# LY-zhang-yi-hao/ORB-SLAM3_byZyh

Hardware: AMD Instinct MI355X
Metric: ORB features/ms (640x480, 8-level) + LocalBA iter ms @1/2/4/8 GPU (higher is better)
Workload: dtype u8; 1 GPU; C2: batch of 64 synthetic 640x480 frames per GPU, nFeatures=1000, 8 levels, extraction+description (ORBextractor::operator()); frames_per_gpu=64, width=640, height=480, nfeatures=1000, nlevels=8, batches_in_flight=4, parallelism=frame-sharded x1

## Files before the change

### orb-slam3_byzyh_amd/csrc/orb_extract.hip

```cpp
#include <hip/hip_ext.h>
#include <hip/hip_runtime.h>

#include <algorithm>
#include <cstdio>
#include <cstdlib>
#include <cstring>
#include <mutex>
#include <string>
#include <type_traits>
#include <vector>

#include "orb_extract_geom.h"
#include "orb_hd.h"
#include "orb_sincos.h"
#include "orbgpu.h"
#include "orbgpu_internal.h"

using namespace orbgpu;

namespace {

constexpr int kPatternSrc[1024] = {
#include "orb_pattern31.inc"
};
// ... 1327 lines not shown

template <bool kKeysInLds>
__device__ void qt2_run(QT2& T, uint32_t* keys, uint16_t* node, int K, int N, int nroots, float root_w, int span_y,
                        const uint32_t* __restrict__ cand_level, const CellDesc* __restrict__ cells, int cell_begin,
                        int cell_count, const int32_t* __restrict__ ccount, int n_first, int slot_first,
                        uint32_t* __restrict__ sel_out, int sel_cap, int* n_sel, int* status, int debug_flags,
                        unsigned long long* stamps, const QPlace& place) {
    QTree& t = T.t;
    const int tid = threadIdx.x, lane = tid & 63, wave = tid >> 6, lcap = t.lcap;
    int* ctrl = T.ctrl;
    unsigned long long* tm = ((debug_flags & 4) && stamps && tid == 0) ? stamps : nullptr;
    if (tm)
        for (int i = 0; i < kQtStamps; ++i) tm[i] = 0;
    unsigned long long t_last = tm ? __builtin_amdgcn_s_memtime() : 0;
    auto stamp = [&](int i) {
        if (tm) { const unsigned long long now = __builtin_amdgcn_s_memtime(); tm[i] += now - t_last; t_last = now; }
    };
    int rcount[kMaxRoots];
#pragma unroll
    for (int r = 0; r < kMaxRoots; ++r) rcount[r] = 0;
    {
        constexpr int kGB = 8;
        int carry = 0;
        for (int cb = 0; cb < cell_count; cb += kQtThreads) {
            const int c = cb + tid;
            int n = 0, slot = 0;
            if (cb == 0) { n = n_first; slot = slot_first; }
            else if (c < cell_count) { n = ccount[c]; slot = cells[cell_begin + c].slot; }
            const int incl = wave_incl_scan(n, lane);
            const int start = incl - n;
            const int Tw = uniform(__builtin_amdgcn_readlane(incl, 63));
            if (lane == 0) ctrl[24 + wave] = Tw;
            __syncthreads();
            int base = carry, tot = 0;
#pragma unroll
            for (int w = 0; w < kQtWaves; ++w) {
                const int v = ctrl[24 + w];
                base += w < wave ? v : 0;
                tot += v;
            }
            __syncthreads();
            for (int j0 = 0; j0 < Tw; j0 += 64 * kGB) {
                uint32_t kk[kGB];
#pragma unroll
                for (int gi = 0; gi < kGB; ++gi) {
                    const int i = j0 + 64 * gi + lane;
                    int cl = 0;
#pragma unroll
                    for (int s = 32; s > 0; s >>= 1)
                        if (__shfl(start, cl + s, 64) <= i) cl += s;
                    const int sl = __shfl(slot, cl, 64), s0 = __shfl(start, cl, 64);
                    kk[gi] = i < Tw ? cand_level[sl + (i - s0)] : 0u;
                }
#pragma unroll
                for (int gi = 0; gi < kGB; ++gi) {
                    const int i = j0 + 64 * gi + lane;
                    if (i < Tw) {
                        int root = 0;
                        if (nroots > 1) {
                            root = (int)((float)key_x(kk[gi]) / root_w);
#pragma unroll
                            for (int r = 0; r < kMaxRoots; ++r) rcount[r] += root == r;
                        }
                        keys[base + i] = kk[gi];
                        node[base + i] = (uint16_t)root;
                    }
                }
            }
            carry += tot;
        }
    }
    if (tid < kMaxRoots) ctrl[16 + tid] = 0;
    __syncthreads();
    if (nroots > 1) {
#pragma unroll
        for (int r = 0; r < kMaxRoots; ++r) {
            if (r >= nroots) break;
            const int s = wave_sum(rcount[r]);
            if (lane == 0 && s) atomicAdd(&ctrl[16 + r], s);
        }
    } else if (tid == 0) {
        ctrl[16] = K;
    }
    __syncthreads();
    stamp(0);
    QGen A = t.g0, B = t.g1;
    int32_t* cA = T.cnt[0];
    int32_t* cB = T.cnt[1];
    uint32_t* sA = T.sxy[0];
    uint32_t* sB = T.sxy[1];
    int nlist = 0;
    if (tid == 0) {
        for (int r = 0; r < nroots; ++r) {
            const int n = ctrl[16 + r];
            if (n > 0) {
                const int x0 = (int)(root_w * (float)r), x1 = (int)(root_w * (float)(r + 1));
                A.x0[nlist] = (int16_t)x0; A.x1[nlist] = (int16_t)x1;
                A.y0[nlist] = 0; A.y1[nlist] = (int16_t)span_y;
                A.kn[nlist] = n; A.leaf[nlist] = n == 1;
                sA[nlist] = n > 1 ? qt2_split_word(x0, 0, x1, span_y) : ~0u;
#pragma unroll
                for (int q = 0; q < 4; ++q) cA[q * lcap + nlist] = 0;
                ctrl[8 + r] = nlist;
                nlist++;
            }
        }
        ctrl[2] = nlist;
    }
    __syncthreads();
    nlist = ctrl[2];
    for (int kb = wave * 64; kb < K; kb += kQtThreads) {
        const int k = kb + lane;
        int p = 0, q = 0;
        bool counted = false;
        if (k < K) {
            if (nroots > 1) {
                p = ctrl[8 + node[k]];
                node[k] = (uint16_t)p;
            }
            const uint32_t s = sA[p];
            counted = s != ~0u;
            q = qt2_quadrant(keys[k], s);
        }
        if (counted) atomicAdd(&cA[q * lcap + p], 1);
    }
    __syncthreads();
    stamp(1);
    bool careful = false, fin = false, ovf = false;
    int nsplit = 0;
    while (true) {
        if (wave == 0) {
            int new_size = 0;
            if (!careful) {
                qt2_regular(T, A, B, cA, cB, sB, nlist, N, lane, new_size, nsplit, fin, ovf);
                if (!fin && !ovf && new_size + nsplit * 3 > N) careful = true;
                stamp(2);
                if (tm) tm[9]++;
            } else {
                if (tm) tm[8] += (unsigned long long)nsplit << (16 * min((int)tm[10], 3));
                qt2_careful(T, A, B, cA, cB, sB, nlist, nsplit, N, lane, debug_flags, K < (1 << 20), new_size, nsplit, fin, ovf, tm,
                            t_last);
                stamp(5);
                if (tm) tm[10]++;
            }
            nlist = new_size;
            if (lane == 0) { ctrl[0] = fin; ctrl[1] = ovf; }
        }
        __syncthreads();
        fin = ctrl[0] != 0;
        ovf = ctrl[1] != 0;
        if (ovf) break;
        for (int kb = wave * 128; kb < K; kb += 2 * kQtThreads) {
            const int k0 = kb + lane, k1 = kb + 64 + lane;
            const bool v0 = k0 < K, v1 = k1 < K;
            const int p0 = v0 ? node[k0] : 0, p1 = v1 ? node[k1] : 0;
            const uint32_t key0 = v0 ? keys[k0] : 0u, key1 = v1 ? keys[k1] : 0u;
            const uint32_t s0 = sA[p0], s1 = sA[p1];
            const unsigned long long m0 = T.cmap[p0], m1 = T.cmap[p1];
            const int n0 = (int)((m0 >> (16 * qt2_quadrant(key0, s0))) & 0xffff);
            const int n1 = (int)((m1 >> (16 * qt2_quadrant(key1, s1))) & 0xffff);
            if (v0) node[k0] = (uint16_t)n0;
            if (v1) node[k1] = (uint16_t)n1;
            if (fin) {
                if (v0) atomicMax(&T.best[n0], ((uint32_t)key_score(key0) << 24) | (0xffffffu - (uint32_t)k0));
                if (v1) atomicMax(&T.best[n1], ((uint32_t)key_score(key1) << 24) | (0xffffffu - (uint32_t)k1));
            } else {
                const uint32_t t0 = v0 ? sB[n0] : ~0u, t1 = v1 ? sB[n1] : ~0u;
                if (t0 != ~0u) atomicAdd(&cB[qt2_quadrant(key0, t0) * lcap + n0], 1);
                if (t1 != ~0u) atomicAdd(&cB[qt2_quadrant(key1, t1) * lcap + n1], 1);
            }
        }
        __syncthreads();
        stamp(careful && !fin ? 6 : 3);
        { const QGen g = A; A = B; B = g; }
        { int32_t* c = cA; cA = cB; cB = c; }
        { uint32_t* s = sA; sA = sB; sB = s; }
        if (fin) break;
    }
    if (wave != 0) return;
    if (ovf || nlist > sel_cap) {
        if (lane == 0) { *n_sel = 0; atomicMax(status, 1); }
        return;
    }
    int carry_lap = 0, carry_mono = 0;
    for (int b = 0; b < nlist; b += 64) {
        const int i = b + lane;
        bool lap = false;
        if (i < nlist) {
            const uint32_t bw = T.best[i];
            const uint32_t best = keys[0xffffffu - (bw & 0xffffffu)];
            sel_out[i] = best;
            float x = (float)(key_x(best) + place.minB);
            if (place.level != 0) x = x * place.scale;
            lap = x >= (float)place.lap0 && x <= (float)place.lap1;
        }
        const unsigned long long ml = ballot(i < nlist && lap), mm = ballot(i < nlist && !lap);
        if (i < nlist) place.rank_out[i] = lap ? -(1 + carry_lap + rank_in(ml)) : carry_mono + rank_in(mm);
        carry_lap += __popcll(ml);
        carry_mono += __popcll(mm);
    }
    if (lane == 0) { *n_sel = nlist; *place.n_lap = carry_lap; }
    stamp(7);
    if (tm) tm[11] = (unsigned long long)K;
}

__global__ __launch_bounds__(kQtThreads) void k_quadtree_kp(
    const KernelGeom* __restrict__ gp, const CellDesc* __restrict__ cells, const uint32_t* __restrict__ cand,
    const int32_t* __restrict__ cell_count, uint32_t* __restrict__ key_scratch, uint32_t* __restrict__ sel,
    int32_t* __restrict__ sel_count, int lds_bytes, int* __restrict__ status, unsigned long long* __restrict__ stamps,
    int lap0, int lap1, int32_t* __restrict__ rank_out, int32_t* __restrict__ lap_count, int level0) {
    const KernelGeom& g = *gp;
    extern __shared__ __attribute__((aligned(16))) uint8_t smem[];
    const int level = level0 + blockIdx.x, f = blockIdx.y, tid = threadIdx.x, lane = tid & 63, wave = tid >> 6;
    const LevelGeom& L = g.lv[level];
    const int32_t* cc = cell_count + (size_t)f * g.ncells + L.cell_begin;
    int32_t* n_sel = sel_count + (size_t)f * g.nlevels + level;
    const int lcap = L.sel_cap + 64;
    const size_t meta = (qt2_meta_bytes(lcap) + 15) & ~(size_t)15;
    if (meta > (size_t)lds_bytes) {
        if (tid == 0) { *n_sel = 0; atomicMax(status, 2); }
        return;
    }
    QT2 T;
    qt2_carve(T, smem, lcap);
    int n_first = 0, slot_first = 0, Kp = 0;
    for (int c = tid; c < L.cell_count; c += kQtThreads) {
        const int v = cc[c];
        if (c == tid) { n_first = v; slot_first = cells[L.cell_begin + c].slot; }
        Kp += v;
    }
    Kp = wave_sum(Kp);
    if (lane == 0) T.ctrl[24 + kQtWaves + wave] = Kp;
    __syncthreads();
    int K = 0;
#pragma unroll
    for (int w = 0; w < kQtWaves; ++w) K += T.ctrl[24 + kQtWaves + w];
    uint32_t* sel_out = sel + (size_t)f * g.sel_frame_cap + L.sel_off;
    const uint32_t* cand_level = cand + (size_t)f * g.cand_frame_cap + L.cand_off;
    QPlace place{level, L.minB, lap0, lap1, L.scale, rank_out + (size_t)f * g.sel_frame_cap + L.sel_off,
                 lap_count + (size_t)f * g.nlevels + level};
    unsigned long long* st = stamps ? stamps + ((size_t)f * g.nlevels + level) * kQtStamps : nullptr;
    if (!(g.debug_flags & 8) && meta + (size_t)K * 6 <= (size_t)lds_bytes) {
        uint32_t* keys = (uint32_t*)(smem + meta);
        uint16_t* node = (uint16_t*)(keys + K);
        qt2_run<true>(T, keys, node, K, L.nfeat, L.n_roots, L.root_w, L.maxBY - L.minB, cand_level, cells,
                      L.cell_begin, L.cell_count, cc, n_first, slot_first, sel_out, L.sel_cap, n_sel, status,
                      g.debug_flags, st, place);
    } else {
        uint32_t* keys = key_scratch + ((size_t)f * g.cand_frame_cap + L.cand_off) * 2;
        uint16_t* node = (uint16_t*)(keys + L.cand_cap);
        qt2_run<false>(T, keys, node, K, L.nfeat, L.n_roots, L.root_w, L.maxBY - L.minB, cand_level, cells,
                       L.cell_begin, L.cell_count, cc, n_first, slot_first, sel_out, L.sel_cap, n_sel, status,
                       g.debug_flags, st, place);
    }
}

__global__ __launch_bounds__(64) void k_debug_node_sort(const int* __restrict__ counts, const int* __restrict__ ulx,
                                                        int n, int mode, int* __restrict__ order, int* __restrict__ used_reg) {
    extern __shared__ __attribute__((aligned(16))) uint8_t smem[];
    QT2 T;
    qt2_carve(T, smem, n + 64);
    QTree& t = T.t;
    QGen& A = t.g0;
    const int lane = threadIdx.x;
    for (int i = lane; i < n; i += 64) { A.kn[i] = counts[i]; A.x0[i] = (int16_t)ulx[i]; t.prev[i] = (uint16_t)i; }
    wave_sync();
    const bool reg = mode == 0 && n <= 64 && qt_sort_reg(t, A, n, lane);
    if (!reg) qt_sort(t, A, n, lane);
    for (int i = lane; i < n; i += 64) order[i] = t.prev[i];
    if (lane == 0) *used_reg = reg;
}

constexpr int kExcPerLane = (kNumSincosExc + 31) / 32;
template <bool kLds = false>
__device__ __forceinline__ void steer_sincos(float ang, const uint32_t (&exc)[kExcPerLane], int half, int hl,
                                             float* s, float* c, const uint2* lds_cs = nullptr) {
    orb_det_sincosf(ang, s, c);
    const uint32_t bits = __float_as_uint(ang);
    int idx = -1;
#pragma unroll
    for (int e = 0; e < kExcPerLane; ++e)
        if (32 * e + hl < kNumSincosExc && exc[e] == bits) idx = 32 * e + hl;
    const uint32_t hm = (uint32_t)(ballot(idx >= 0) >> (32 * (half & 1)));
    if (hm) {
        const int hit = __shfl(idx, 32 * (half & 1) + __builtin_ctz(hm), 64);
        if constexpr (kLds) {
            *c = __uint_as_float(lds_cs[hit].x);
            *s = __uint_as_float(lds_cs[hit].y);
        } else {
            *c = __uint_as_float(c_sincos_exc[hit][1]);
            *s = __uint_as_float(c_sincos_exc[hit][2]);
        }
    }
}

constexpr int kDescKpPerBlock = 8;
constexpr int kPR = 43, kPRW = 12;
constexpr int kHP = 22, kHPW = 40;
constexpr int kDescWords = kHP * kHPW;
static_assert(kDescWords >= (kPR + 1) * kPRW + 1, "patch + the last pair's odd row and over-read word fit the region");

typedef float f32x2 __attribute__((ext_vector_type(2)));
constexpr f32x2 kRound2 = {12582912.0f, 12582912.0f};
constexpr int kRoundBits = 0x4B400000;

__device__ __forceinline__ int blur_sample(const uint32_t* __restrict__ H, int r, int c) {
    const unsigned i = (unsigned)(r + 18) & 63u, cc = (unsigned)(c + 18) & 63u;
    const uint32_t* p = H + __umul24(i >> 1, (unsigned)kHPW) + cc;
    const bool odd = (i & 1) != 0;
    uint32_t acc = 1u << 15;
    acc = __builtin_amdgcn_udot2(as_u16x2(p[0]), odd ? w16(0, 18) : w16(18, 34), acc, false);
    acc = __builtin_amdgcn_udot2(as_u16x2(p[kHPW]), odd ? w16(34, 48) : w16(48, 56), acc, false);
    acc = __builtin_amdgcn_udot2(as_u16x2(p[2 * kHPW]), odd ? w16(56, 48) : w16(48, 34), acc, false);
    acc = __builtin_amdgcn_udot2(as_u16x2(p[3 * kHPW]), odd ? w16(34, 18) : w16(18, 0), acc, false);
    return (int)(acc >> 16);
}

__global__ __launch_bounds__(256) void k_describe(const KernelGeom* __restrict__ gp, const uint8_t* __restrict__ pyr,
                                                  const uint32_t* __restrict__ sel,
                                                  const int32_t* __restrict__ sel_count,
                                                  const int32_t* __restrict__ rank_in_class, const int32_t* __restrict__ lap_count,
                                                  int cap, orb_keypoint_t* __restrict__ kps, uint8_t* __restrict__ desc,
                                                  int32_t* __restrict__ counts, int chunks, int nblocks, int share,
                                                  int stage_levels, int stage_mode, orb_keypoint_t* __restrict__ st_kp,
                                                  uint8_t* __restrict__ st_desc) {
    const KernelGeom& g = *gp;
    __shared__ __attribute__((aligned(16))) uint32_t patch[kDescKpPerBlock][kDescWords];
    const int half = threadIdx.x >> 5, hl = threadIdx.x & 31;
    const int tb = xcd_tile(blockIdx.x, share);
    if (tb >= nblocks) return;
    const int f = tb / chunks, chunk0 = tb - f * chunks;
    int level = 0, chunk = chunk0;
#pragma unroll
    for (int l = 0; l + 1 < kMaxLevels; ++l) {
        const int c = (g.lv[l].sel_cap + kDescKpPerBlock - 1) / kDescKpPerBlock;
        if (l + 1 < g.nlevels && level == l && chunk >= c) { chunk -= c; level = l + 1; }
    }
    const int slot = chunk * kDescKpPerBlock + half;
    const LevelGeom& L = g.lv[level];
    const size_t sbase = (size_t)f * g.sel_frame_cap + L.sel_off + (slot < L.sel_cap ? slot : L.sel_cap - 1);
    const uint32_t key_spec = L.sel_cap > 0 ? sel[sbase] : 0u;
    const int rk_spec = L.sel_cap > 0 ? rank_in_class[sbase] : 0;
    const int li = hl & 15;
    const int cnt_l = li < g.nlevels ? sel_count[(size_t)f * g.nlevels + li] : 0;
    const int lap_l = li < g.nlevels ? lap_count[(size_t)f * g.nlevels + li] : 0;
    uint32_t pat[8], exc[kExcPerLane], disc[16];
#pragma unroll
    for (int m = 0; m < 8; ++m) pat[m] = c_pattern_packed.w[32 * m + hl];
#pragma unroll
    for (int m = 0; m < 16; ++m) disc[m] = c_disc.w[hl][m];
#pragma unroll
    for (int e = 0; e < kExcPerLane; ++e) exc[e] = 32 * e + hl < kNumSincosExc ? c_sincos_exc[32 * e + hl][0] : 0u;
    int total = cnt_l, lap_before = li < level ? lap_l : 0, mono_before = li < level ? cnt_l - lap_l : 0;
    total = row16_isum(total);
    lap_before = row16_isum(lap_before);
    mono_before = row16_isum(mono_before);
    const int n = __shfl(cnt_l, (threadIdx.x & ~15) + level, 64);
    const size_t st_idx = sbase;
    if (stage_mode != 1 && chunk0 == 0 && threadIdx.x == 0) {
        int mono = 0;
        for (int l = 0; l < g.nlevels; ++l)
            mono += sel_count[(size_t)f * g.nlevels + l] - lap_count[(size_t)f * g.nlevels + l];
        counts[2 * f] = total;
        counts[2 * f + 1] = total > cap ? ORB_ERR_CAPACITY : mono;
    }
    if (chunk * kDescKpPerBlock >= n) return;
    const bool active = slot < n && (stage_mode == 1 || total <= cap);
    if (stage_mode == 2 && level < stage_levels) {
        if (!active) return;
        const int rk = rk_spec;
        const int dst = rk < 0 ? total - 1 - (lap_before + (-rk - 1)) : mono_before + rk;
        if (hl < 8)
            reinterpret_cast<uint32_t*>(desc + ((size_t)f * cap + dst) * 32)[hl] =
                reinterpret_cast<const uint32_t*>(st_desc + st_idx * 32)[hl];
        else if (hl == 8)
            kps[(size_t)f * cap + dst] = st_kp[st_idx];
        return;
    }
    const uint32_t key = active ? key_spec : 0;
    const int x = key_x(key) + L.minB, y = key_y(key) + L.minB;
    constexpr int kGroups = (kPR + 9) / 10;
    const int pr = hl / 3, pq = hl - 3 * pr;
    const uint8_t* up = pyr + (size_t)f * g.pyr_frame_bytes + L.plane_off;
    const int po = (y + kEdge - 21) * L.pitch + (x + kEdge - 21);
    const int sh = po & 3;
    const uint32_t vo = (uint32_t)(po - sh + pr * L.pitch + 16 * pq);
    const __amdgpu_buffer_rsrc_t ru = __builtin_amdgcn_make_buffer_rsrc(const_cast<uint8_t*>(up), (short)0, 0x7fffffff, kBufDword3);
    uint32_t* P = patch[half];
    if (active && hl < 30) {
        v4u32 v[kGroups];
#pragma unroll
        for (int k = 0; k < kGroups; ++k) v[k] = __builtin_amdgcn_raw_buffer_load_b128(ru, vo, 10 * k * L.pitch, 0);
#pragma unroll
        for (int k = 0; k < kGroups; ++k)
            if (10 * k + pr < kPR) *reinterpret_cast<v4u32*>(P + (10 * k + pr) * kPRW + 4 * pq) = v[k];
    }
    wave_sync();
    int m10 = 0, m01 = 0;
    {
        const int rb = sh + (hl + 6) * (kPRW * 4) + 6;
        const uint32_t* rw = P + (rb >> 2);
        const int ra = rb & 3;
        uint32_t d[9];
#pragma unroll
        for (int k = 0; k < 9; ++k) d[k] = rw[k];
        uint32_t S = 0, W = 0;
#pragma unroll
        for (int k = 0; k < 8; ++k) {
            const uint32_t x = __builtin_amdgcn_alignbyte(d[k + 1], d[k], ra);
            S = __builtin_amdgcn_udot4(x, disc[k], S, false);
            W = __builtin_amdgcn_udot4(x, disc[8 + k], W, false);
        }
        if (active && hl < 31) {
            m01 = (hl - 15) * (int)S;
            m10 = (int)W - 16 * (int)S;
        }
    }
    m10 = half_wave_sum(m10);
    m01 = half_wave_sum(m01);
    const float angle = orb_fast_atan2((float)m01, (float)m10);
    constexpr int kItems = kHP * 10, kIt = (kItems + 31) / 32;
#pragma unroll
    for (int it = kIt - 1; it >= 0; --it) {
        const int i = hl + 32 * it, ic = min(i, kItems - 1), j = ic / 10, qq = ic - 10 * j;
        uint32_t o[2][4];
#pragma unroll
        for (int rr = 0; rr < 2; ++rr) {
            const uint32_t* w = P + (2 * j + rr) * kPRW + qq;
            const uint32_t w0 = w[0], w1 = w[1], w2 = w[2], w3 = w[3];
            const uint32_t a0 = __builtin_amdgcn_alignbyte(w1, w0, sh);
            const uint32_t a1 = __builtin_amdgcn_alignbyte(w2, w1, sh);
            const uint32_t a2 = __builtin_amdgcn_alignbyte(w3, w2, sh);
            o[rr][0] = __builtin_amdgcn_udot4(a1, kBlurK1, __builtin_amdgcn_udot4(a0, kBlurK0, 0u, false), false);
            o[rr][1] = __builtin_amdgcn_udot4(a1, kBlurS1[1], __builtin_amdgcn_udot4(a0, kBlurS0[1], 0u, false), false);
            o[rr][2] = __builtin_amdgcn_udot4(a2, kBlurS2[2], __builtin_amdgcn_udot4(a1, kBlurS1[2],
                                              __builtin_amdgcn_udot4(a0, kBlurS0[2], 0u, false), false), false);
            o[rr][3] = __builtin_amdgcn_udot4(a2, kBlurS2[3], __builtin_amdgcn_udot4(a1, kBlurS1[3],
                                              __builtin_amdgcn_udot4(a0, kBlurS0[3], 0u, false), false), false);
        }
        if (i < kItems)
            *reinterpret_cast<uint4*>(P + j * kHPW + 4 * qq) =
                make_uint4(o[0][0] | o[1][0] << 16, o[0][1] | o[1][1] << 16, o[0][2] | o[1][2] << 16, o[0][3] | o[1][3] << 16);
    }
    wave_sync();
    const float ang = angle * (float)(3.14159265358979323846 / 180.f);
    float a, b;
    steer_sincos(ang, exc, half, hl, &b, &a);
    int t0[8], t1[8];
#pragma unroll
    for (int m = 0; m < 8; ++m) {
        const int pw4 = (int)pat[m];
        const float px0 = (float)((pw4 << 24) >> 24), py0 = (float)((pw4 << 16) >> 24);
        const float px1 = (float)((pw4 << 8) >> 24), py1 = (float)(pw4 >> 24);
        const f32x2 rc0 = __builtin_elementwise_fma(f32x2{px0, px0}, f32x2{b, a}, f32x2{py0, py0} * f32x2{a, -b}) + kRound2;
        const f32x2 rc1 = __builtin_elementwise_fma(f32x2{px1, px1}, f32x2{b, a}, f32x2{py1, py1} * f32x2{a, -b}) + kRound2;
        t0[m] = blur_sample(P, __float_as_int(rc0.x) - kRoundBits, __float_as_int(rc0.y) - kRoundBits);
        t1[m] = blur_sample(P, __float_as_int(rc1.x) - kRoundBits, __float_as_int(rc1.y) - kRoundBits);
    }
    uint32_t words[8];
#pragma unroll
    for (int m = 0; m < 8; ++m) words[m] = (uint32_t)(ballot(t0[m] < t1[m]) >> (32 * (half & 1)));
    if (!active) return;
    const int rk = rk_spec;
    const int dst = rk < 0 ? total - 1 - (lap_before + (-rk - 1)) : mono_before + rk;
    uint8_t* drow = stage_mode == 1 ? st_desc + st_idx * 32 : desc + ((size_t)f * cap + dst) * 32;
    orb_keypoint_t* kdst = stage_mode == 1 ? st_kp + st_idx : kps + (size_t)f * cap + dst;
    if (hl < 8) {
        uint32_t w = words[0];
#pragma unroll
        for (int m = 1; m < 8; ++m) if (hl == m) w = words[m];
        reinterpret_cast<uint32_t*>(drow)[hl] = w;
    } else if (hl == 8) {
        orb_keypoint_t k;
        float fx = (float)x, fy = (float)y;
        if (level != 0) { fx = fx * L.scale; fy = fy * L.scale; }
        k.x = fx; k.y = fy;
        k.size = (float)L.patch_size;
        k.angle = angle;
        k.response = (float)key_score(key);
        k.octave = level;
        k.class_id = -1;
        *kdst = k;
    }
}

}

namespace orbgpu {

enum { kLaunchPyramid = 0, kLaunchFast = 1, kLaunchQuadtree = 2, kLaunchDescribe = 3 };

struct Extractor {
    Params P;
    int max_w = 0, max_h = 0, max_batch = 0;
    int cur_w = -1, cur_h = -1;
    Geometry geo;
    bool geo_ok = false;
    orbgpu::KernelGeom* d_geom = nullptr;
    CellDesc* d_cells = nullptr; size_t cells_cap = 0;
    int2* d_xtab = nullptr; size_t xtab_cap = 0;
    int4* d_tiletab = nullptr; size_t tiletab_cap = 0;
    int4* d_pairtab = nullptr; size_t pairtab_cap = 0;
    bool pair_ok = false;
    int pyr_pair = 0;
    int tile_off[orbgpu::kMaxLevels] = {};
    int4* d_ytab = nullptr; size_t ytab_cap = 0;
    uint8_t* d_pyr = nullptr; size_t pyr_cap = 0;
    uint32_t* d_cand = nullptr; size_t cand_cap = 0;
    uint32_t* d_scratch = nullptr; size_t scratch_cap = 0;
    int32_t* d_cell_count = nullptr; size_t cell_count_cap = 0;
    uint8_t* d_cell_thr = nullptr; size_t cell_thr_cap = 0;
    uint32_t* d_sel = nullptr; size_t sel_cap = 0;
    int32_t* d_dst = nullptr; size_t dst_cap = 0;
    int32_t* d_sel_count = nullptr; size_t selcount_cap = 0;
    int32_t* d_lap_count = nullptr; size_t lapcount_cap = 0;
    int* d_status = nullptr;
    int* d_status_own = nullptr;
    bool clear_status_l0 = false;
    uint8_t* d_img = nullptr; size_t img_cap = 0;
    uint8_t* d_out = nullptr; uint8_t* h_out = nullptr;
    orb_keypoint_t* d_kps = nullptr; uint8_t* d_desc = nullptr; int32_t* d_counts = nullptr; size_t out_cap = 0;
    hipGraph_t g1_graph = nullptr;
    hipGraphExec_t g1_exec = nullptr;
    std::vector<uintptr_t> g1_key;
    hipStream_t stream = nullptr;
    int last_n = 0;
    int qt_lds = 0;
    static constexpr int kMaxStreams = 4;
    int chunk = 1 << 30, nstreams = 1;
    bool fast_stamps = false, pyr_stamps = false;
    int fast_split = 3;
    int fast_split_cfg = 3;
    int chain_fast_split = 1;
    int qt_key_room = 4;
    int pyr_affine = 1;
    int ablate = 0;
    int fast_per_level = 0;
    int desc_split = 1;
    orb_keypoint_t* d_st_kp = nullptr; size_t st_kp_cap = 0;
    uint8_t* d_st_desc = nullptr; size_t st_desc_cap = 0;
    int qt_split = 0;
    hipStream_t side = nullptr, side2 = nullptr;
    hipEvent_t split_ev[3] = {};
    hipEvent_t lvl_ev[orbgpu::kMaxLevels] = {};
    hipStream_t sub[kMaxStreams] = {};
    hipEvent_t fork_ev = nullptr, join_ev[kMaxStreams] = {};
    long long batches = 0;
    int profile = 0;
    std::vector<hipEvent_t> pyr_events;
    size_t pyr_ev_used = 0;
    std::vector<int> pyr_ev_kernel;
    std::vector<hipEvent_t> events;
    int ev_used = 0;
    long long frames_profiled = 0;
    unsigned long long* d_stamps = nullptr;
    size_t stamps_cap = 0;
};

}

using orbgpu::Extractor;

namespace {

template <class T>
int grow(T*& p, size_t& cap, size_t need) {
    if (need <= cap && p) return ORB_OK;
    if (p) (void)hipFree(p);
    p = nullptr;
    cap = 0;
    if (need == 0) need = 1;
    if (hipMalloc(&p, need * sizeof(T)) != hipSuccess) { p = nullptr; return orbgpu_fail(ORB_ERR_DEVICE, "hipMalloc failed"); }
    cap = need;
    return ORB_OK;
}

int pyr_tiles_x(const orbgpu::LevelGeom& L) { return (L.w + 2 * kBorder + kTileW - 1) / kTileW; }
int pyr_tiles_y(const orbgpu::LevelGeom& L) { return (L.h + 2 * kBorder + kTileH - 1) / kTileH; }
void tile_tables(const orbgpu::KernelGeom& k, std::vector<int4>& tab, int* off) {
    auto refl = [](int a, int b, int len, int& lo, int& hi) {
        lo = 1 << 30; hi = -1;
        if (a < 0) { const int e2 = std::min(b, -1); lo = std::min(lo, -e2); hi = std::max(hi, -a); }
        if (b >= 0 && a < len) { lo = std::min(lo, std::max(a, 0)); hi = std::max(hi, std::min(b, len - 1)); }
        if (b >= len) { const int s0 = std::max(a, len); lo = std::min(lo, 2 * len - 2 - b); hi = std::max(hi, 2 * len - 2 - s0); }
    };
    auto src = [](int d, double scale, int slen) {
        const float f = (float)((d + 0.5) * scale - 0.5);
        int s2 = (int)f;
        s2 -= (s2 > f);
        return std::min(std::max(s2, 0), slen - 1);
    };
    tab.clear();
    for (int l = 0; l < k.nlevels; ++l) {
        const orbgpu::LevelGeom& L = k.lv[l];
        off[l] = (int)tab.size();
        for (int ty = 0; ty < pyr_tiles_y(L); ++ty)
            for (int tx = 0; tx < pyr_tiles_x(L); ++tx) {
                const int X0 = kEdge - kBorder + tx * kTileW, Y0 = kEdge - kBorder + ty * kTileH;
                int4 r = make_int4(X0 | Y0 << 16, 0, 0, 0);
                if (l > 0) {
                    const orbgpu::LevelGeom& P = k.lv[l - 1];
                    const double scx = 1. / ((double)L.w / P.w), scy = 1. / ((double)L.h / P.h);
                    int a, b;
                    refl(X0 - kEdge, std::min(X0 + kTileW - 1 - kEdge, L.w + kBorder - 1), L.w, a, b);
                    const int bx0 = src(a, scx, P.w), bw = std::min(src(b, scx, P.w) + 1, P.w - 1) - bx0 + 1;
                    refl(Y0 - kEdge, std::min(Y0 + kTileH - 1 - kEdge, L.h + kBorder - 1), L.h, a, b);
                    const int by0 = src(a, scy, P.h), bh = std::min(src(b, scy, P.h) + 1, P.h - 1) - by0 + 1;
                    r.y = bx0 | bw << 16;
                    r.z = by0 | bh << 16;
                }
                tab.push_back(r);
            }
    }
}

bool pair_tables(const orbgpu::KernelGeom& k, const std::vector<int4>& tiles, const int* off, std::vector<int4>& tab) {
    auto src = [](int d, double scale, int slen) {
        const float f = (float)((d + 0.5) * scale - 0.5);
        int s2 = (int)f;
        s2 -= (s2 > f);
        return std::min(std::max(s2, 0), slen - 1);
    };
    auto refl = [](int p, int len) { p = p < 0 ? -p : p; return p >= len ? 2 * len - 2 - p : p; };
    tab.assign(2 * tiles.size(), make_int4(0, 0, 0, 0));
    for (int nl = 1; nl < k.nlevels; nl += 2) {
        const orbgpu::LevelGeom &N = k.lv[nl], &L = k.lv[nl - 1];
        const int ntx = pyr_tiles_x(N), nty = pyr_tiles_y(N);
        std::vector<int> cx(ntx + 1), cy(nty + 1);
        cx[0] = -kBorder; cx[ntx] = L.w + kBorder;
        cy[0] = -kBorder; cy[nty] = L.h + kBorder;
        for (int i = 1; i < ntx; ++i) cx[i] = tiles[off[nl] + i].y & 0xffff;
        for (int j = 1; j < nty; ++j) cy[j] = tiles[off[nl] + j * ntx].z & 0xffff;
        for (int i = 0; i < ntx; ++i) if (cx[i] >= cx[i + 1]) return false;
        for (int j = 0; j < nty; ++j) if (cy[j] >= cy[j + 1]) return false;
        for (int ty = 0; ty < nty; ++ty)
            for (int tx = 0; tx < ntx; ++tx) {
                const int idx = off[nl] + ty * ntx + tx;
                const int4 T = tiles[idx];
                int ux0 = T.y & 0xffff, ux1 = ux0 + (T.y >> 16), uy0 = T.z & 0xffff, uy1 = uy0 + (T.z >> 16);
                const int ox0 = cx[tx], ox1 = cx[tx + 1], oy0 = cy[ty], oy1 = cy[ty + 1];
                for (int x = ox0; x < ox1; ++x) { const int v = refl(x, L.w); ux0 = std::min(ux0, v); ux1 = std::max(ux1, v + 1); }
                for (int y = oy0; y < oy1; ++y) { const int v = refl(y, L.h); uy0 = std::min(uy0, v); uy1 = std::max(uy1, v + 1); }
                const int uw = ux1 - ux0, uh = uy1 - uy0;
                const int nch = ((ox1 + kEdge - 1) >> 3) - ((ox0 + kEdge) >> 3) + 1;
                if (uw + 8 > kPairUP || uw > 128 + 32 || uh > kPairUH || nch > 21 || ox0 < -32768 || ox1 > 32767) return false;
                int cx0 = 0, cw = 0, cy0 = 0, chh = 0;
                if (nl > 1) {
                    const orbgpu::LevelGeom& Pv = k.lv[nl - 2];
                    const double scx = 1. / ((double)L.w / Pv.w), scy = 1. / ((double)L.h / Pv.h);
                    cx0 = src(ux0, scx, Pv.w);
                    cw = std::min(src(ux1 - 1, scx, Pv.w) + 1, Pv.w - 1) - cx0 + 1;
                    cy0 = src(uy0, scy, Pv.h);
                    chh = std::min(src(uy1 - 1, scy, Pv.h) + 1, Pv.h - 1) - cy0 + 1;
                    if (cw + 3 + 8 > kPairCW || chh > kPairCH) return false;
                }
                tab[2 * idx] = make_int4(ux0 | uw << 16, uy0 | uh << 16, cx0 | cw << 16, cy0 | chh << 16);
                tab[2 * idx + 1] = make_int4((ox0 & 0xffff) | ox1 << 16, (oy0 & 0xffff) | oy1 << 16, 0, 0);
            }
    }
    return true;
}

int prepare(Extractor* e, int w, int h, int n) {
    if (w != e->cur_w || h != e->cur_h) {
        if (e->cur_w >= 0 && hipDeviceSynchronize() != hipSuccess) return orbgpu_fail(ORB_ERR_DEVICE, "sync failed");
        orbgpu::Geometry g;
        if (!orbgpu::build_geometry(e->P, w, h, g)) return orbgpu_fail(ORB_ERR_ARG, "image too small for the pyramid/cell grid");
        for (int v = 0; v < 16; ++v)
            if (g.k.umax[v] != kDiscUmax[v]) return orbgpu_fail(ORB_ERR_INTERNAL, "umax differs from the IC_Angle disc table");
        e->geo = g;
        e->cur_w = w;
        e->cur_h = h;
        int rc;
        if ((rc = grow(e->d_cells, e->cells_cap, g.cells.size())) != ORB_OK) return rc;
        if ((rc = grow(e->d_xtab, e->xtab_cap, std::max<size_t>(1, g.xtab.size() / 2))) != ORB_OK) return rc;
        if ((rc = grow(e->d_ytab, e->ytab_cap, std::max<size_t>(1, g.ytab.size() / 4))) != ORB_OK) return rc;
        if (!e->d_geom && hipMalloc(&e->d_geom, sizeof(orbgpu::KernelGeom)) != hipSuccess)
            return orbgpu_fail(ORB_ERR_DEVICE, "hipMalloc failed");
        if (hipMemcpy(e->d_geom, &g.k, sizeof(orbgpu::KernelGeom), hipMemcpyHostToDevice) != hipSuccess ||
            hipMemcpy(e->d_cells, g.cells.data(), g.cells.size() * sizeof(orbgpu::CellDesc), hipMemcpyHostToDevice) != hipSuccess ||
            (!g.xtab.empty() && hipMemcpy(e->d_xtab, g.xtab.data(), g.xtab.size() * 4, hipMemcpyHostToDevice) != hipSuccess) ||
            (!g.ytab.empty() && hipMemcpy(e->d_ytab, g.ytab.data(), g.ytab.size() * 4, hipMemcpyHostToDevice) != hipSuccess))
            return orbgpu_fail(ORB_ERR_DEVICE, "table upload failed");
        std::vector<int4> tt;
        tile_tables(g.k, tt, e->tile_off);
        for (int l = 1; l < g.k.nlevels; ++l) {
            const bool small = 4 * g.k.lv[l - 1].w <= 5 * g.k.lv[l].w && 4 * g.k.lv[l - 1].h <= 5 * g.k.lv[l].h;
            const int bwmax = (small ? kSmallBoxW : kBoxW) - 3, bhmax = small ? kSmallBoxH : kBoxH;
            const int t1 = l + 1 < g.k.nlevels ? e->tile_off[l + 1] : (int)tt.size();
            for (int t = e->tile_off[l]; t < t1; ++t)
                if ((tt[t].y >> 16) > bwmax || (tt[t].z >> 16) > bhmax) {
                    e->cur_w = e->cur_h = -1;
                    e->geo_ok = false;
                    return orbgpu_fail(ORB_ERR_ARG, "pyramid level ratio above 2 (scale factor too large)");
                }
        }
        if ((rc = grow(e->d_tiletab, e->tiletab_cap, tt.size())) != ORB_OK) return rc;
        if (hipMemcpy(e->d_tiletab, tt.data(), tt.size() * sizeof(int4), hipMemcpyHostToDevice) != hipSuccess)
            return orbgpu_fail(ORB_ERR_DEVICE, "table upload failed");
        std::vector<int4> pt;
        e->pair_ok = pair_tables(g.k, tt, e->tile_off, pt);
        if (e->pair_ok) {
            if ((rc = grow(e->d_pairtab, e->pairtab_cap, pt.size())) != ORB_OK) return rc;
            if (hipMemcpy(e->d_pairtab, pt.data(), pt.size() * sizeof(int4), hipMemcpyHostToDevice) != hipSuccess)
                return orbgpu_fail(ORB_ERR_DEVICE, "table upload failed");
        }
        e->geo_ok = true;
        size_t meta = 0;
        for (int l = 0; l < g.k.nlevels; ++l) {
            const int lcap = g.k.lv[l].sel_cap + 64;
            meta = std::max(meta, (qt2_meta_bytes(lcap) + 15) & ~(size_t)15);
        }
        const size_t want = meta + (size_t)e->qt_key_room * 1024;
        if (meta > 160 * 1024) return orbgpu_fail(ORB_ERR_ARG, "nfeatures too large for the quad-tree LDS budget");
        e->qt_lds = (int)std::min<size_t>(want, 160 * 1024);
        if (hipFuncSetAttribute((const void*)k_quadtree_kp, hipFuncAttributeMaxDynamicSharedMemorySize, 160 * 1024) !=
            hipSuccess)
            return orbgpu_fail(ORB_ERR_DEVICE, "cannot raise the quad-tree LDS limit");
    }
    const orbgpu::KernelGeom& k = e->geo.k;
    int rc;
    if ((rc = grow(e->d_pyr, e->pyr_cap, (size_t)k.pyr_frame_bytes * n)) != ORB_OK) return rc;
    if ((rc = grow(e->d_cand, e->cand_cap, (size_t)k.cand_frame_cap * n)) != ORB_OK) return rc;
    if ((rc = grow(e->d_scratch, e->scratch_cap, (size_t)k.cand_frame_cap * n * 2)) != ORB_OK) return rc;
    if ((rc = grow(e->d_cell_count, e->cell_count_cap, (size_t)k.ncells * n)) != ORB_OK) return rc;
    if ((rc = grow(e->d_cell_thr, e->cell_thr_cap, (size_t)k.ncells * n)) != ORB_OK) return rc;
    if ((rc = grow(e->d_sel, e->sel_cap, (size_t)k.sel_frame_cap * n)) != ORB_OK) return rc;
    if ((rc = grow(e->d_dst, e->dst_cap, (size_t)k.sel_frame_cap * n)) != ORB_OK) return rc;
    if ((rc = grow(e->d_sel_count, e->selcount_cap, (size_t)k.nlevels * n)) != ORB_OK) return rc;
    if ((rc = grow(e->d_lap_count, e->lapcount_cap, (size_t)k.nlevels * n)) != ORB_OK) return rc;
    if (e->desc_split) {
        if ((rc = grow(e->d_st_kp, e->st_kp_cap, (size_t)k.sel_frame_cap * n)) != ORB_OK) return rc;
        if ((rc = grow(e->d_st_desc, e->st_desc_cap, (size_t)k.sel_frame_cap * n * 32)) != ORB_OK) return rc;
    }
    if ((k.debug_flags & 4) && (rc = grow(e->d_stamps, e->stamps_cap, (size_t)k.nlevels * n * kQtStamps)) != ORB_OK) return rc;
    return ORB_OK;
}

int launch_chunk(Extractor* e, int f0, const uint8_t* d_images, int n, int stride, size_t frame_stride, int lap0,
                 int lap1, orb_keypoint_t* d_kps, uint8_t* d_desc, int cap, int32_t* d_counts, hipStream_t st) {
    const orbgpu::Geometry& G = e->geo;
    const orbgpu::KernelGeom& k = G.k;
    hipEvent_t* ev = nullptr;
    if (e->profile == 1 || e->profile == 2) {
        const size_t need = (size_t)(e->ev_used + 1) * (orbgpu::kStages + 1);
        while (e->events.size() < need) {
            hipEvent_t x;
            if (hipEventCreate(&x) != hipSuccess) return orbgpu_fail(ORB_ERR_DEVICE, "hipEventCreate failed");
            e->events.push_back(x);
        }
        ev = &e->events[(size_t)e->ev_used * (orbgpu::kStages + 1)];
        e->ev_used++;
        e->frames_profiled += n;
    }
    auto mark = [&](int i) {
        if (ev && (e->profile == 1 || (e->profile == 2 && i <= 1))) hipEventRecord(ev[i], st);
    };
    uint8_t* pyr = e->d_pyr + (size_t)f0 * k.pyr_frame_bytes;
    uint32_t* cand = e->d_cand + (size_t)f0 * k.cand_frame_cap;
    uint32_t* scratch = e->d_scratch + (size_t)f0 * k.cand_frame_cap * 2;
    int32_t* ccount = e->d_cell_count + (size_t)f0 * k.ncells;
    uint8_t* cthr = e->d_cell_thr + (size_t)f0 * k.ncells;
    uint32_t* sel = e->d_sel + (size_t)f0 * k.sel_frame_cap;
    int32_t* dst = e->d_dst + (size_t)f0 * k.sel_frame_cap;
    int32_t* scount = e->d_sel_count + (size_t)f0 * k.nlevels;
    int32_t* lapc = e->d_lap_count + (size_t)f0 * k.nlevels;
    const uint8_t* imgs = d_images + (size_t)f0 * frame_stride;
    orb_keypoint_t* kps = d_kps + (size_t)f0 * cap;
    uint8_t* desc = d_desc + (size_t)f0 * cap * 32;
    int32_t* counts = d_counts + 2 * (size_t)f0;
    mark(0);
    const int split = (n > 1 && e->fast_split > 0 && e->fast_split < k.nlevels) ? e->fast_split : 0;
    const bool fast_stamps = e->fast_stamps;
    auto launch_events = [&](int kernel) -> hipEvent_t* {
// ... 713 lines not shown
```

Baseline: 362,400 features/ms.

## Compact describe blur to reachable patch items and streamline sampling and ballots

The horizontal-blur pass in k_describe now iterates over a compile-time table holding only the patch items the rBRIEF pattern can reach (189 of 220, six rounds instead of seven), with static_asserts that check coverage and in-place safety. Blur sampling is rewritten to use raw LDS addresses with alignbit, removing the odd/even row select, and ballots are moved into lanes with v_writelane instead of a per-lane select chain. The atan2 is replaced by a local polynomial version. Together these aim to cut LDS traffic and ALU work per keypoint, at the cost of inline asm and address-space tricks that are harder to maintain.

```diff
diff --git a/orb-slam3_byzyh_amd/csrc/orb_extract.hip b/orb-slam3_byzyh_amd/csrc/orb_extract.hip
--- a/orb-slam3_byzyh_amd/csrc/orb_extract.hip
+++ b/orb-slam3_byzyh_amd/csrc/orb_extract.hip
@@ -1653,17 +1653,131 @@
 
 typedef float f32x2 __attribute__((ext_vector_type(2)));
 constexpr f32x2 kRound2 = {12582912.0f, 12582912.0f};
-constexpr int kRoundBits = 0x4B400000;
-
-__device__ __forceinline__ int blur_sample(const uint32_t* __restrict__ H, int r, int c) {
-    const unsigned i = (unsigned)(r + 18) & 63u, cc = (unsigned)(c + 18) & 63u;
-    const uint32_t* p = H + __umul24(i >> 1, (unsigned)kHPW) + cc;
-    const bool odd = (i & 1) != 0;
+constexpr uint32_t kRoundBits = 0x4B400000u;
+
+constexpr int pattern_r2_max() {
+    int m = 0;
+    for (int k = 0; k < 512; ++k) {
+        const int x = kPatternSrc[2 * k], y = kPatternSrc[2 * k + 1], d = x * x + y * y;
+        if (x < -18 || x > 18 || y < -18 || y > 18) return -1;
+        m = d > m ? d : m;
+    }
+    return m;
+}
+constexpr int kPatR2 = pattern_r2_max();
+static_assert(kPatR2 == 338, "rBRIEF pattern radius: the patch (43 x 43) and the sums (43 x 37) are sized for 18 px");
+constexpr bool sample_reachable(int r, int c) {
+    const int u = 2 * (r < 0 ? -r : r) - 1, v = 2 * (c < 0 ? -c : c) - 1;
+    return (u > 0 ? u * u : 0) + (v > 0 ? v * v : 0) <= 4 * kPatR2 + 1;
+}
+struct HItemNeed { bool need[kHP][10]; int n; };
+constexpr HItemNeed hitem_need() {
+    HItemNeed t{};
+    for (int r = -18; r <= 18; ++r)
+        for (int c = -18; c <= 18; ++c)
+            if (sample_reachable(r, c))
+                for (int k = 0; k < 7; ++k) t.need[(r + 18 + k) >> 1][(c + 18) >> 2] = true;
+    for (int j = 0; j < kHP; ++j)
+        for (int q = 0; q < 10; ++q) t.n += t.need[j][q];
+    return t;
+}
+constexpr int kHItems = hitem_need().n, kHRounds = (kHItems + 31) / 32;
+struct HItemTable { uint32_t w[kHRounds][32]; };
+constexpr uint32_t hitem_word(int j, int q) { return (uint32_t)(4 * (2 * j * kPRW + q)) | (uint32_t)(4 * (j * kHPW + 4 * q)) << 16; }
+constexpr HItemTable make_hitems() {
+    const HItemNeed nd = hitem_need();
+    HItemTable t{};
+    int n = 0;
+    uint32_t last = 0;
+    for (int j = kHP - 1; j >= 0; --j)
+        for (int q = 9; q >= 0; --q)
+            if (nd.need[j][q]) { last = hitem_word(j, q); t.w[n >> 5][n & 31] = last; ++n; }
+    for (; n < kHRounds * 32; ++n) t.w[n >> 5][n & 31] = last;
+    return t;
+}
+constexpr bool hitems_cover() {
+    const HItemTable t = make_hitems();
+    bool wr[kHP][10] = {};
+    for (int i = 0; i < kHRounds * 32; ++i) {
+        const int o = (int)(t.w[i >> 5][i & 31] >> 16) / 4;
+        wr[o / kHPW][(o % kHPW) / 4] = true;
+    }
+    for (int r = -18; r <= 18; ++r)
+        for (int c = -18; c <= 18; ++c)
+            if (sample_reachable(r, c))
+                for (int k = 0; k < 7; ++k)
+                    if (!wr[(r + 18 + k) >> 1][(c + 18) >> 2]) return false;
+    return true;
+}
+constexpr bool hitems_in_place() {
+    const HItemTable t = make_hitems();
+    for (int a = 0; a < kHRounds * 32; ++a) {
+        const int wa = (int)(t.w[a >> 5][a & 31] >> 16);
+        if (wa + 16 > 4 * kDescWords) return false;
+        for (int b = (a | 31) + 1; b < kHRounds * 32; ++b) {
+            const int rb = (int)(t.w[b >> 5][b & 31] & 0xffff);
+            for (int rr = 0; rr < 2; ++rr)
+                if (wa < rb + 4 * rr * kPRW + 16 && rb + 4 * rr * kPRW < wa + 16) return false;
+        }
+    }
+    return true;
+}
+static_assert(kHItems == 189 && kHRounds == 6, "items a sample can reach (of 22 x 10): six rounds of 32 lanes");
+static_assert(hitems_cover(), "every reachable sample's 7 sum rows are produced");
+static_assert(hitems_in_place(), "the compacted order never reads a patch byte that an earlier round overwrote");
+__constant__ HItemTable c_hitems = make_hitems();
+
+typedef __attribute__((address_space(3))) uint32_t lds_u32;
+__device__ __forceinline__ uint32_t lds_addr(const uint32_t* p) { return (uint32_t)(uintptr_t)(const lds_u32*)p; }
+__device__ __forceinline__ lds_u32* lds_at(uint32_t a) { return (lds_u32*)(uintptr_t)a; }
+
+__device__ __forceinline__ float describe_atan2(float y, float x) {
+    const float k = (float)(180 / 3.14159265358979323846);
+    const float p1 = 0.9997878412794807f * k, p3 = -0.3258083974640975f * k;
+    const float p5 = 0.1555786518463281f * k, p7 = -0.04432655554792128f * k;
+    const float eps = (float)2.220446049250313080847e-16;
+    const float ax = x < 0 ? -x : x, ay = y < 0 ? -y : y;
+    const bool flat = ax >= ay;
+    const float c = (flat ? ay : ax) / ((flat ? ax : ay) + eps), c2 = c * c;
+    const float p = (((p7 * c2 + p5) * c2 + p3) * c2 + p1) * c;
+    float a = flat ? p : 90.f - p;
+    if (x < 0) a = 180.f - a;
+    if (y < 0) a = 360.f - a;
+    return a;
+}
+
+__device__ __forceinline__ uint32_t ballots_to_lanes(const unsigned long long (&b)[8]) {
+    uint32_t w = 0;
+    asm("s_nop 1\n\t"
+        "v_writelane_b32 %0, %1, 0\n\tv_writelane_b32 %0, %2, 32\n\t"
+        "v_writelane_b32 %0, %3, 1\n\tv_writelane_b32 %0, %4, 33\n\t"
+        "v_writelane_b32 %0, %5, 2\n\tv_writelane_b32 %0, %6, 34\n\t"
+        "v_writelane_b32 %0, %7, 3\n\tv_writelane_b32 %0, %8, 35\n\t"
+        "v_writelane_b32 %0, %9, 4\n\tv_writelane_b32 %0, %10, 36\n\t"
+        "v_writelane_b32 %0, %11, 5\n\tv_writelane_b32 %0, %12, 37\n\t"
+        "v_writelane_b32 %0, %13, 6\n\tv_writelane_b32 %0, %14, 38\n\t"
+        "v_writelane_b32 %0, %15, 7\n\tv_writelane_b32 %0, %16, 39"
+        : "+v"(w)
+        : "s"((uint32_t)b[0]), "s"((uint32_t)(b[0] >> 32)), "s"((uint32_t)b[1]), "s"((uint32_t)(b[1] >> 32)),
+          "s"((uint32_t)b[2]), "s"((uint32_t)(b[2] >> 32)), "s"((uint32_t)b[3]), "s"((uint32_t)(b[3] >> 32)),
+          "s"((uint32_t)b[4]), "s"((uint32_t)(b[4] >> 32)), "s"((uint32_t)b[5]), "s"((uint32_t)(b[5] >> 32)),
+          "s"((uint32_t)b[6]), "s"((uint32_t)(b[6] >> 32)), "s"((uint32_t)b[7]), "s"((uint32_t)(b[7] >> 32)));
+    return w;
+}
+
+__device__ __forceinline__ uint32_t blur_base(uint32_t region) {
+    return region + 4u * (9u * kHPW + 18u) - 0x400000u * (2u * kHPW) - (kRoundBits << 2);
+}
+__device__ __forceinline__ int blur_sample(uint32_t base, uint32_t rb, uint32_t cb) {
+    uint32_t row = __umul24(rb & ~1u, 2u * kHPW) + base;
+    asm("" : "+v"(row));
+    const lds_u32* p = lds_at((cb << 2) + row);
+    const uint32_t s = rb << 4, p0 = p[0], p1 = p[kHPW], p2 = p[2 * kHPW], p3 = p[3 * kHPW];
     uint32_t acc = 1u << 15;
-    acc = __builtin_amdgcn_udot2(as_u16x2(p[0]), odd ? w16(0, 18) : w16(18, 34), acc, false);
-    acc = __builtin_amdgcn_udot2(as_u16x2(p[kHPW]), odd ? w16(34, 48) : w16(48, 56), acc, false);
-    acc = __builtin_amdgcn_udot2(as_u16x2(p[2 * kHPW]), odd ? w16(56, 48) : w16(48, 34), acc, false);
-    acc = __builtin_amdgcn_udot2(as_u16x2(p[3 * kHPW]), odd ? w16(34, 18) : w16(18, 0), acc, false);
+    acc = __builtin_amdgcn_udot2(as_u16x2(__builtin_amdgcn_alignbit(p1, p0, s)), w16(18, 34), acc, false);
+    acc = __builtin_amdgcn_udot2(as_u16x2(__builtin_amdgcn_alignbit(p2, p1, s)), w16(48, 56), acc, false);
+    acc = __builtin_amdgcn_udot2(as_u16x2(__builtin_amdgcn_alignbit(p3, p2, s)), w16(48, 34), acc, false);
+    acc = __builtin_amdgcn_udot2(as_u16x2(__builtin_amdgcn_alignbit(p3, p3, s)), w16(18, 0), acc, false);
     return (int)(acc >> 16);
 }
 
@@ -1695,9 +1809,11 @@
     const int li = hl & 15;
     const int cnt_l = li < g.nlevels ? sel_count[(size_t)f * g.nlevels + li] : 0;
     const int lap_l = li < g.nlevels ? lap_count[(size_t)f * g.nlevels + li] : 0;
-    uint32_t pat[8], exc[kExcPerLane], disc[16];
+    uint32_t pat[8], exc[kExcPerLane], disc[16], hit[kHRounds];
 #pragma unroll
     for (int m = 0; m < 8; ++m) pat[m] = c_pattern_packed.w[32 * m + hl];
+#pragma unroll
+    for (int it = 0; it < kHRounds; ++it) hit[it] = c_hitems.w[it][hl];
 #pragma unroll
     for (int m = 0; m < 16; ++m) disc[m] = c_disc.w[hl][m];
 #pragma unroll
@@ -1769,15 +1885,15 @@
     }
     m10 = half_wave_sum(m10);
     m01 = half_wave_sum(m01);
-    const float angle = orb_fast_atan2((float)m01, (float)m10);
-    constexpr int kItems = kHP * 10, kIt = (kItems + 31) / 32;
-#pragma unroll
-    for (int it = kIt - 1; it >= 0; --it) {
-        const int i = hl + 32 * it, ic = min(i, kItems - 1), j = ic / 10, qq = ic - 10 * j;
+    const float angle = describe_atan2((float)m01, (float)m10);
+    const uint32_t region = lds_addr(P);
+#pragma unroll
+    for (int it = 0; it < kHRounds; ++it) {
+        const lds_u32* src = lds_at(region + (hit[it] & 0xffffu));
         uint32_t o[2][4];
 #pragma unroll
         for (int rr = 0; rr < 2; ++rr) {
-            const uint32_t* w = P + (2 * j + rr) * kPRW + qq;
+            const lds_u32* w = src + rr * kPRW;
             const uint32_t w0 = w[0], w1 = w[1], w2 = w[2], w3 = w[3];
             const uint32_t a0 = __builtin_amdgcn_alignbyte(w1, w0, sh);
             const uint32_t a1 = __builtin_amdgcn_alignbyte(w2, w1, sh);
@@ -1789,14 +1905,17 @@
             o[rr][3] = __builtin_amdgcn_udot4(a2, kBlurS2[3], __builtin_amdgcn_udot4(a1, kBlurS1[3],
                                               __builtin_amdgcn_udot4(a0, kBlurS0[3], 0u, false), false), false);
         }
-        if (i < kItems)
-            *reinterpret_cast<uint4*>(P + j * kHPW + 4 * qq) =
-                make_uint4(o[0][0] | o[1][0] << 16, o[0][1] | o[1][1] << 16, o[0][2] | o[1][2] << 16, o[0][3] | o[1][3] << 16);
+        lds_u32* dstw = lds_at(region + (hit[it] >> 16));
+        uint32_t pk[4];
+#pragma unroll
+        for (int k = 0; k < 4; ++k) pk[k] = __builtin_amdgcn_perm(o[1][k], o[0][k], 0x05040100u);
+        *reinterpret_cast<__attribute__((address_space(3))) v4u32*>(dstw) = v4u32{pk[0], pk[1], pk[2], pk[3]};
     }
     wave_sync();
     const float ang = angle * (float)(3.14159265358979323846 / 180.f);
     float a, b;
     steer_sincos(ang, exc, half, hl, &b, &a);
+    const uint32_t bbase = blur_base(region);
     int t0[8], t1[8];
 #pragma unroll
     for (int m = 0; m < 8; ++m) {
@@ -1805,22 +1924,20 @@
         const float px1 = (float)((pw4 << 8) >> 24), py1 = (float)(pw4 >> 24);
         const f32x2 rc0 = __builtin_elementwise_fma(f32x2{px0, px0}, f32x2{b, a}, f32x2{py0, py0} * f32x2{a, -b}) + kRound2;
         const f32x2 rc1 = __builtin_elementwise_fma(f32x2{px1, px1}, f32x2{b, a}, f32x2{py1, py1} * f32x2{a, -b}) + kRound2;
-        t0[m] = blur_sample(P, __float_as_int(rc0.x) - kRoundBits, __float_as_int(rc0.y) - kRoundBits);
-        t1[m] = blur_sample(P, __float_as_int(rc1.x) - kRoundBits, __float_as_int(rc1.y) - kRoundBits);
-    }
-    uint32_t words[8];
-#pragma unroll
-    for (int m = 0; m < 8; ++m) words[m] = (uint32_t)(ballot(t0[m] < t1[m]) >> (32 * (half & 1)));
+        t0[m] = blur_sample(bbase, __float_as_uint(rc0.x), __float_as_uint(rc0.y));
+        t1[m] = blur_sample(bbase, __float_as_uint(rc1.x), __float_as_uint(rc1.y));
+    }
+    unsigned long long bal[8];
+#pragma unroll
+    for (int m = 0; m < 8; ++m) bal[m] = ballot(t0[m] < t1[m]);
+    const uint32_t word = ballots_to_lanes(bal);
     if (!active) return;
     const int rk = rk_spec;
     const int dst = rk < 0 ? total - 1 - (lap_before + (-rk - 1)) : mono_before + rk;
     uint8_t* drow = stage_mode == 1 ? st_desc + st_idx * 32 : desc + ((size_t)f * cap + dst) * 32;
     orb_keypoint_t* kdst = stage_mode == 1 ? st_kp + st_idx : kps + (size_t)f * cap + dst;
     if (hl < 8) {
-        uint32_t w = words[0];
-#pragma unroll
-        for (int m = 1; m < 8; ++m) if (hl == m) w = words[m];
-        reinterpret_cast<uint32_t*>(drow)[hl] = w;
+        reinterpret_cast<uint32_t*>(drow)[hl] = word;
     } else if (hl == 8) {
         orb_keypoint_t k;
         float fx = (float)x, fy = (float)y;
```

New measurement: 375,900 features/ms, median of 6. 3.7% higher.
